# 0xEigenLabs/eigen-zkvm

Hardware: AMD Instinct MI355X
Metric: Goldilocks NTT GElems/s + BN254 G1 MSM Mpts/s; starky prove ms at 2^24 rows (higher is better)
Workload: dtype u64 (Goldilocks, canonical)

## Files before the change

eigen-zkvm_amd/csrc/ntt.hip:

```cpp
#include "zk_internal.h"
#include "ntt_reg.hip.h"
#include <map>
#include <mutex>
#include <type_traits>
#include <vector>

namespace zk {

namespace {

constexpr int NTT_TILE = 4096;
constexpr int TW_LO_BITS = 12;
constexpr int TW_LO = 1 << TW_LO_BITS;

struct PassParams {
    const u64* in;
    u64* out;
    const u64* w256;
    const u64* tw_lo;
    const u64* tw_hi;
    const u64* tw_mid;
    u64 pre_scale;
    u32 dshift;
    const u64* sc_lo;
    const u64* sc_hi;
    u64 sc_step;
    u64 out_scale;
    u64 inner;
    u64 valid_in;
    u64 s_np;
    u32 np;
    u32 log_s;
    u32 has_tw;
};

__device__ __forceinline__ u64 tab2(const u64* __restrict__ lo, const u64* __restrict__ hi, u64 e) {
    return gl::mul_tw_nc(hi[e >> TW_LO_BITS], lo[e & (TW_LO - 1)]);
}

template <int LOGA, int LOGB, bool KMODE, bool INV>
__global__ __launch_bounds__(NTT_TILE / 16) void ntt_pass_kernel(const PassParams P) {
    constexpr int LOGR = LOGA + LOGB, R = 1 << LOGR, RA = 1 << LOGA, RB = 1 << LOGB;
    constexpr int C = NTT_TILE / R;
    constexpr int GA = 16 / RA, GB = 16 / RB;
    constexpr int TG = R / 16;
    constexpr int PAD = KMODE ? 512 / R : 0;
    constexpr int ROW = RB * C + PAD;
    static_assert(LOGR >= 4 && LOGR <= 8 && LOGA <= 4 && LOGB <= 4, "tile shape");
    __shared__ u64 lds[RA * ROW];

    const int t = threadIdx.x;
    const u64 u0 = (u64)blockIdx.x * C;

    {
        const int c = t % C, ta = t / C;
        const u64 u = u0 + c;
        const bool live = u < P.inner;
        u64 x[GA][RA];
        const bool full = u0 + C <= P.inner && (u64)(R - 1) * P.inner + u0 + C <= P.valid_in;
        const u64* __restrict__ base = P.in + (u64)(ta * GA) * P.inner + (live ? u : 0);
        if (full) {
#pragma unroll
            for (int g = 0; g < GA; ++g)
#pragma unroll
                for (int ja = 0; ja < RA; ++ja) x[g][ja] = __builtin_nontemporal_load(&base[(u64)(ja * RB + g) * P.inner]);
        } else {
#pragma unroll
            for (int g = 0; g < GA; ++g)
#pragma unroll
                for (int ja = 0; ja < RA; ++ja) {
                    const u64 off = (u64)(ja * RB + g) * P.inner;
                    const bool ok = live && (u64)(ta * GA) * P.inner + off + u < P.valid_in;
                    const u64 v = __builtin_nontemporal_load(ok ? base + off : P.in);
                    x[g][ja] = ok ? v : 0;
                }
        }
#pragma unroll
        for (int g = 0; g < GA; ++g) ntt_reg<LOGA, INV>(x[g]);
        if (LOGR <= 6 && C >= 64 && LOGB > 0 && P.pre_scale == 1) {
            static_for<0, TG>([&](auto TA) {
                constexpr int ta_c = decltype(TA)::value;
                if (ta == ta_c) {
                    static_for<0, GA>([&](auto GI) {
                        constexpr int g = decltype(GI)::value, jb = ta_c * GA + g;
                        static_for<0, RA>([&](auto KA) {
                            constexpr int ka = decltype(KA)::value;
                            constexpr int e0 = (39 * (64 / (R > 64 ? 64 : R)) * jb * ka) % 192, e = INV ? (192 - e0) % 192 : e0;
                            u64 v = x[g][bitrev_c(ka, LOGA)];
                            if constexpr (e >= 96) v = gl::neg(gl::mul_pow2<e - 96>(v));
                            else v = gl::mul_pow2<e>(v);
                            lds[ka * ROW + jb * C + c] = v;
                        });
                    });
                }
            });
        } else
        {
#pragma unroll
            for (int g = 0; g < GA; ++g) {
                const int jb = ta * GA + g;
#pragma unroll
                for (int ka = 0; ka < RA; ++ka) {
                    u64 v = x[g][bitrev_c(ka, LOGA)];
                    if (LOGB > 0 && ka > 0) v = gl::mul_tw(v, P.w256[(jb * ka) << (8 - LOGR)]);
                    else if (P.pre_scale != 1) v = gl::mul_tw(v, P.pre_scale);
                    lds[ka * ROW + jb * C + c] = v;
                }
            }
        }
    }
    __syncthreads();
    {
        int c, tb;
        if (KMODE) { tb = t % TG; c = t / TG; } else { c = t % C; tb = t / C; }
        const u64 u = u0 + c;
        u64 y[GB][RB];
#pragma unroll
        for (int g = 0; g < GB; ++g) {
            const int ka = tb + g * TG;
#pragma unroll
            for (int jb = 0; jb < RB; ++jb) y[g][jb] = lds[ka * ROW + jb * C + c];
        }
        const u64 uc = u < P.inner ? u : 0;
        u64 p, rem;
        if (P.np == 1) { p = uc >> P.log_s; rem = uc & (((u64)1 << P.log_s) - 1); }
        else if ((P.inner >> 32) == 0) { const u32 p32 = (u32)uc / (u32)P.s_np; p = p32; rem = (u32)uc - p32 * (u32)P.s_np; }
        else
        { p = uc / P.s_np; rem = uc - p * P.s_np; }
        u64 tw[GB][RB];
        if (P.tw_mid) {
            const u32 sh = P.log_s - P.dshift, istep = (((u32)p * RA) << sh) * 8;
#pragma unroll
            for (int g = 0; g < GB; ++g) {
                const u32 ka = tb + g * TG, i0 = (((u32)p * ka) << sh) * 8;
#pragma unroll
                for (int kb = 0; kb < RB; ++kb) tw[g][kb] = *(const u64*)((const char*)P.tw_mid + (u32)(i0 + kb * istep));
            }
        }
#pragma unroll
        for (int g = 0; g < GB; ++g) ntt_reg<LOGB, INV>(y[g]);
        if (u >= P.inner) return;

        auto finish = [&](auto small_c) {
            constexpr bool SMALL = decltype(small_c)::value;
            u64* __restrict__ outp = P.out + p * R * P.s_np + rem;
            const u64 kstride = P.s_np;
            const u32 b0 = ((u32)p * R * (u32)P.s_np + (u32)rem) * 8, bstep = RA * (u32)P.s_np * 8;
            auto put = [&](u32 ka, int kb, u64 v) {
                if constexpr (SMALL) *(u64*)((char*)P.out + (u32)(b0 + ka * (u32)P.s_np * 8 + kb * bstep)) = v;
                else outp[(u64)(RA * kb + ka) * kstride] = v;
            };
            const u64 row_q = !P.sc_lo ? 0 : P.np == 1 ? rem : (P.inner >> 32) == 0 ? (u64)((u32)rem / P.np) : rem / P.np;
            if (P.tw_mid) {
#pragma unroll
                for (int g = 0; g < GB; ++g) {
                    const int ka = tb + g * TG;
#pragma unroll
                    for (int kb = 0; kb < RB; ++kb) {
                        u64 v = y[g][bitrev_c(kb, LOGB)];
                        v = gl::mul_tw(v, tw[g][kb]);
                        put(ka, kb, v);
                    }
                }
                return;
            }
            u64 tw_step = 1;
            if (P.has_tw) tw_step = tab2(P.tw_lo, P.tw_hi, (p * RA) << P.log_s);
#pragma unroll
            for (int g = 0; g < GB; ++g) {
                const int ka = tb + g * TG;
                u64 f = P.out_scale;
                if (P.has_tw) f = tab2(P.tw_lo, P.tw_hi, (p * ka) << P.log_s);
                if (P.sc_lo) f = tab2(P.sc_lo, P.sc_hi, ((u64)ka << P.log_s) + row_q);
                const bool scaled = P.has_tw || P.sc_lo || P.out_scale != 1;
                const u64 fstep = P.sc_lo ? P.sc_step : tw_step;
#pragma unroll
                for (int kb = 0; kb < RB; ++kb) {
                    u64 v = y[g][bitrev_c(kb, LOGB)];
                    if (scaled) {
                        v = gl::mul_tw(v, f);
                        if (kb + 1 < RB) f = gl::mul_tw_nc(f, fstep);
                    }
                    put(ka, kb, v);
                }
            }
        };
        if (((P.inner * R) >> 29) == 0) finish(std::true_type{});
        else finish(std::false_type{});
    }
}

__global__ void ntt_small_kernel(const u64* in, u64* out, u32 np, u32 n_in, u32 n, u64 w, u64 g, u64 cst) {
    const u32 tid = blockIdx.x * blockDim.x + threadIdx.x;
    if (tid >= n * np) return;
    const u32 k = tid / np, c = tid % np;
    const u64 wk = gl::pow(w, k);
    u64 acc = 0, cur = 1;
    for (u32 i = 0; i < n_in; ++i) { acc = gl::add(acc, gl::mul(in[(u64)i * np + c], cur)); cur = gl::mul(cur, wk); }
    out[(u64)k * np + c] = gl::mul(acc, gl::mul(cst, gl::pow(g, k)));
}

struct Tables { DevConst w256, w256s, lo, hi, mid; u32 dshift = 0; };
struct ScaleTables { DevConst lo, hi; };

std::mutex g_mu;
auto& g_tables = *new std::map<std::pair<int, std::pair<u32, int>>, Tables>;
auto& g_scales = *new std::map<std::pair<int, std::pair<u32, u64>>, ScaleTables>;

void two_level(u64 base, u64 cst, u32 nbits, std::vector<u64>& lo, std::vector<u64>& hi) {
    lo.resize(TW_LO);
    u64 c = cst;
    for (int i = 0; i < TW_LO; ++i) { lo[i] = c; c = gl::hmul(c, base); }
    size_t nh = nbits > (u32)TW_LO_BITS ? (size_t)1 << (nbits - TW_LO_BITS) : 1;
    hi.resize(nh);
    u64 step = gl::hpow(base, TW_LO);
    c = 1;
    for (size_t i = 0; i < nh; ++i) { hi[i] = c; c = gl::hmul(c, step); }
}

const Tables& get_tables(u32 nbits, bool inverse) {
    int dev; ZK_HIP(hipGetDevice(&dev));
    std::lock_guard<std::mutex> lk(g_mu);
    auto key = std::make_pair(dev, std::make_pair(nbits, (int)inverse));
    auto it = g_tables.find(key);
    if (it != g_tables.end()) return it->second;
    u64 w = gl::hroot(nbits), w8 = gl::hroot(8);
    if (inverse) { w = gl::hinv(w); w8 = gl::hinv(w8); }
    std::vector<u64> t256(256), lo, hi;
    u64 c = 1;
    for (int i = 0; i < 256; ++i) { t256[i] = c; c = gl::hmul(c, w8); }
    two_level(w, 1, nbits, lo, hi);
    Tables T; T.w256 = DevConst(t256); T.lo = DevConst(lo); T.hi = DevConst(hi);
    if (inverse) {
        const u64 ninv = gl::hinv((1ull << nbits) % GL_P);
        std::vector<u64> t256s(256);
        for (int i = 0; i < 256; ++i) t256s[i] = gl::hmul(t256[i], ninv);
        T.w256s = DevConst(t256s);
    }
    {
        T.dshift = nbits > 16 ? nbits - 16 : 0;
        const size_t nm = (size_t)1 << (nbits - T.dshift);
        std::vector<u64> mid(nm);
        const u64 step = gl::hpow(w, 1ull << T.dshift);
        c = 1;
        for (size_t i = 0; i < nm; ++i) { mid[i] = c; c = gl::hmul(c, step); }
        T.mid = DevConst(mid);
    }
    return g_tables.emplace(key, std::move(T)).first->second;
}

const ScaleTables& get_scale(u32 nbits, u64 g, u64 cst) {
    int dev; ZK_HIP(hipGetDevice(&dev));
    std::lock_guard<std::mutex> lk(g_mu);
    auto key = std::make_pair(dev, std::make_pair(nbits, g));
    auto it = g_scales.find(key);
    if (it != g_scales.end()) return it->second;
    std::vector<u64> lo, hi;
    two_level(g, cst, nbits, lo, hi);
    ScaleTables S; S.lo = DevConst(lo); S.hi = DevConst(hi);
    return g_scales.emplace(key, std::move(S)).first->second;
}

template <int LOGA, int LOGB>
void launch_pass(const PassParams& P, bool kmode, bool inverse, hipStream_t st) {
    constexpr int C = NTT_TILE >> (LOGA + LOGB);
    const u64 blocks = (P.inner + C - 1) / C;
    ZK_REQUIRE(blocks < (1ull << 31), "ntt: grid too large");
    const dim3 g((u32)blocks), b(NTT_TILE / 16);
    const int variant = (kmode ? 2 : 0) | (inverse ? 1 : 0);
#define ZK_PASS(K, I) hipLaunchKernelGGL((ntt_pass_kernel<LOGA, LOGB, K, I>), g, b, 0, st, P)
    switch (variant) {
        case 0: ZK_PASS(false, false); break; case 1: ZK_PASS(false, true); break;
        case 2: ZK_PASS(true, false); break;  default: ZK_PASS(true, true); break;
    }
#undef ZK_PASS
    ZK_HIP(hipGetLastError());
}

void launch_pass_logr(int logr, const PassParams& P, bool kmode, bool inverse, hipStream_t st) {
    switch (logr) {
        case 4: launch_pass<2, 2>(P, kmode, inverse, st); break;
        case 5: launch_pass<3, 2>(P, kmode, inverse, st); break;
        case 6: launch_pass<3, 3>(P, kmode, inverse, st); break;
        case 7: launch_pass<4, 3>(P, kmode, inverse, st); break;
        case 8: launch_pass<4, 4>(P, kmode, inverse, st); break;
        default: throw Error("ntt: unsupported pass radix");
    }
}

std::vector<int> plan(u32 nbits) {
    std::vector<int> r;
    if (nbits < 4) return r;
    int np = (nbits + 7) / 8;
    int base = nbits / np, extra = nbits % np;
    for (int i = 0; i < np; ++i) r.push_back(base + (i < extra ? 1 : 0));
    return r;
}

struct Scale { bool on = false; u64 g = 1, cst = 1; };

void run_transform(const u64* in, u64* a, u64* b,
                   u32 n_pols, u32 nbits, u64 valid_rows, bool inverse, Scale sc, u64 out_scale, hipStream_t st) {
    const u64 n = 1ull << nbits;
    if (nbits < 4) {
        u64 w = gl::hroot(nbits);
        if (inverse) w = gl::hinv(w);
        u64 cst = sc.on ? sc.cst : out_scale;
        u64 g = sc.on ? sc.g : 1;
        u32 total = (u32)(n * n_pols);
        hipLaunchKernelGGL(ntt_small_kernel, dim3((total + 255) / 256), dim3(256), 0, st, in, a, n_pols,
                           (u32)valid_rows, (u32)n, w, g, cst);
        ZK_HIP(hipGetLastError());
        return;
    }
    const std::vector<int> radices = plan(nbits);
    const int np = (int)radices.size();
    const Tables& T = get_tables(nbits, inverse);
    const ScaleTables* S = sc.on ? &get_scale(nbits, sc.g, sc.cst) : nullptr;
    u32 log_s = 0;
    const u64* cur = in;
    for (int i = 0; i < np; ++i) {
        const int logr = radices[i];
        u64* dstbuf = ((np - 1 - i) % 2 == 0) ? a : b;
        const bool last = (i == np - 1);
        PassParams P{};
        P.in = cur; P.out = dstbuf;
        P.w256 = T.w256.u(); P.tw_lo = T.lo.u(); P.tw_hi = T.hi.u();
        P.sc_lo = (last && sc.on) ? S->lo.u() : nullptr;
        P.sc_hi = (last && sc.on) ? S->hi.u() : nullptr;
        const int loga = (logr + 1) / 2;
        P.sc_step = (last && sc.on) ? gl::hpow(sc.g, (1ull << loga) << log_s) : 1;
        P.out_scale = 1; P.pre_scale = 1;
        if (last && !sc.on && out_scale != 1) {
            ZK_REQUIRE(inverse && out_scale == gl::hinv(n % GL_P), "ntt: unsupported constant scaling");
            P.w256 = T.w256s.u(); P.pre_scale = out_scale;
        }
        P.inner = (n >> logr) * n_pols;
        P.valid_in = (i == 0) ? valid_rows * n_pols : n * n_pols;
        P.s_np = ((u64)1 << log_s) * n_pols;
        P.np = n_pols;
        P.log_s = log_s;
        P.has_tw = last ? 0 : 1;
        P.dshift = T.dshift;
        P.tw_mid = (!last && log_s >= T.dshift) ? T.mid.u() : nullptr;
        const bool kmode = P.s_np < 16;
        launch_pass_logr(logr, P, kmode, inverse, st);
        cur = dstbuf;
        log_s += logr;
    }
}

}

int ntt_num_passes(uint32_t nbits) { return nbits < 4 ? 1 : (int)plan(nbits).size(); }

const u64* ntt_w256_table(bool inverse) { return get_tables(8, inverse).w256.u(); }

void ntt_dev(const u64* d_src, u64* d_dst, u64* d_tmp, uint32_t n_pols, uint32_t nbits, bool inverse, hipStream_t st) {
    ZK_REQUIRE(nbits <= 32, "ntt: nbits > 32");
    if (n_pols == 0) return;
    ZK_REQUIRE(d_src != d_dst, "ntt: dst may not alias src");
    u64 out_scale = inverse ? gl::hinv((1ull << nbits) % GL_P) : 1;
    run_transform(d_src, d_dst, d_tmp, n_pols, nbits, 1ull << nbits, inverse, Scale{}, out_scale, st);
}

void lde_dev(const u64* d_src, u64* d_dst, u64* d_tmp, uint32_t n_pols, uint32_t nbits, uint32_t nbits_ext, hipStream_t st) {
    ZK_REQUIRE(nbits_ext <= 32 && nbits <= nbits_ext, "lde: need nbits <= nbits_ext <= 32");
    if (n_pols == 0) return;
    ZK_REQUIRE(d_src != d_dst, "lde: dst may not alias src");
    const u64 n = 1ull << nbits;
    Scale sc; sc.on = true; sc.g = 49; sc.cst = gl::hinv(n % GL_P);
    const int fwd_passes = ntt_num_passes(nbits_ext);
    u64* first_fwd_out = ((fwd_passes - 1) % 2 == 0) ? d_dst : d_tmp;
    u64* coef = (first_fwd_out == d_dst) ? d_tmp : d_dst;
    u64* other = (coef == d_dst) ? d_tmp : d_dst;
    run_transform(d_src, coef, other, n_pols, nbits, n, true, sc, 1, st);
    run_transform(coef, d_dst, d_tmp, n_pols, nbits_ext, n, false, Scale{}, 1, st);
}

}
```

Before: 94.52.

## Share twiddle loads across 16-lane rows via DPP broadcast and prefetch tables early

In the NTT pass kernel, each lane of a 16-lane row now loads one distinct w256 or tw_mid twiddle, and the row gets the value it needs through DPP row broadcasts. This replaces the per-lane redundant table gathers, used when the row shares the same p (s_np a multiple of 16, non-K mode). The twiddle and scale table lookups for the output chain are also issued before the first-stage register NTT and the barrier, so their latency overlaps compute. The cost is extra register pressure from the prefetched values and DPP cross-lane instructions. It also relies on the assumption that all 16 lanes in a row share p.

```diff
diff --git a/eigen-zkvm_amd/csrc/ntt.hip b/eigen-zkvm_amd/csrc/ntt.hip
--- a/eigen-zkvm_amd/csrc/ntt.hip
+++ b/eigen-zkvm_amd/csrc/ntt.hip
@@ -32,10 +32,17 @@
     u32 np;
     u32 log_s;
     u32 has_tw;
+    u32 row_p;
 };
 
-__device__ __forceinline__ u64 tab2(const u64* __restrict__ lo, const u64* __restrict__ hi, u64 e) {
-    return gl::mul_tw_nc(hi[e >> TW_LO_BITS], lo[e & (TW_LO - 1)]);
+__device__ __forceinline__ u32 dpp_opaque(u32 v) { asm volatile("" : "+v"(v)); return v; }
+template <int SRC>
+__device__ __forceinline__ u64 row_bcast(u64 v) {
+    static_assert(SRC >= 0 && SRC < 16, "a lane of the row");
+    const u32 v0 = dpp_opaque((u32)v), v1 = dpp_opaque((u32)(v >> 32));
+    const u32 z0 = dpp_opaque((u32)__builtin_amdgcn_update_dpp(0, (int)v0, 0x150 + SRC, 0xF, 0xF, false));
+    const u32 z1 = dpp_opaque((u32)__builtin_amdgcn_update_dpp(0, (int)v1, 0x150 + SRC, 0xF, 0xF, false));
+    return gl::mk64(z0, z1);
 }
 
 template <int LOGA, int LOGB, bool KMODE, bool INV>
@@ -52,6 +59,49 @@
     const int t = threadIdx.x;
     const u64 u0 = (u64)blockIdx.x * C;
 
+    auto lane_pos = [&](int c, u64& p, u64& rem) {
+        const u64 u = u0 + c, uc = u < P.inner ? u : 0;
+        if (P.np == 1) { p = uc >> P.log_s; rem = uc & (((u64)1 << P.log_s) - 1); }
+        else if ((P.inner >> 32) == 0) { const u32 p32 = (u32)uc / (u32)P.s_np; p = p32; rem = (u32)uc - p32 * (u32)P.s_np; }
+        else
+        { p = uc / P.s_np; rem = uc - p * P.s_np; }
+    };
+    const int cb = KMODE ? t / TG : t % C, tb = KMODE ? t % TG : t / C;
+
+    static_assert(C % 16 == 0 && GA * RA == 16 && GB * RB == 16, "a 16-lane row shares ta and owns 16 table entries");
+    const int r16 = t & 15;
+    const bool shift_a = LOGR <= 6 && C >= 64 && LOGB > 0 && P.pre_scale == 1;
+    u64 wa = 0;
+    u64 wm = 0;
+    const bool row_p = !KMODE && P.row_p;
+    const bool chain_tab = !P.tw_mid && (P.has_tw || P.sc_lo);
+    u64 f0[GB], tw_step = 1, t2h[GB + 1], t2l[GB + 1];
+    auto request_tables = [&]() {
+        if (LOGB > 0 && !shift_a) wa = P.w256[(((t / C) * GA + r16 / RA) * (r16 % RA)) << (8 - LOGR)];
+        if (row_p) {
+            u64 p, rem;
+            lane_pos(cb & ~15, p, rem);
+            const u32 kappa = tb + (r16 / RB) * TG + RA * (r16 % RB);
+            wm = *(const u64*)((const char*)P.tw_mid + (u32)((((u32)p * kappa) << (P.log_s - P.dshift)) * 8));
+        }
+        if (chain_tab) {
+            u64 p, rem;
+            lane_pos(cb, p, rem);
+            const u64 row_q = !P.sc_lo ? 0 : P.np == 1 ? rem : (P.inner >> 32) == 0 ? (u64)((u32)rem / P.np) : rem / P.np;
+            const u64 es = (p * RA) << P.log_s;
+            t2h[GB] = P.has_tw ? P.tw_hi[es >> TW_LO_BITS] : 1; t2l[GB] = P.has_tw ? P.tw_lo[es & (TW_LO - 1)] : 1;
+            const u64* __restrict__ hi = P.sc_lo ? P.sc_hi : P.tw_hi;
+            const u64* __restrict__ lo = P.sc_lo ? P.sc_lo : P.tw_lo;
+#pragma unroll
+            for (int g = 0; g < GB; ++g) {
+                const int ka = tb + g * TG;
+                const u64 e = P.sc_lo ? ((u64)ka << P.log_s) + row_q : (p * ka) << P.log_s;
+                t2h[g] = hi[e >> TW_LO_BITS]; t2l[g] = lo[e & (TW_LO - 1)];
+            }
+        }
+    };
+    u64 tw[GB][RB];
+
     {
         const int c = t % C, ta = t / C;
         const u64 u = u0 + c;
@@ -75,9 +125,10 @@
                     x[g][ja] = ok ? v : 0;
                 }
         }
+        request_tables();
 #pragma unroll
         for (int g = 0; g < GA; ++g) ntt_reg<LOGA, INV>(x[g]);
-        if (LOGR <= 6 && C >= 64 && LOGB > 0 && P.pre_scale == 1) {
+        if (shift_a) {
             static_for<0, TG>([&](auto TA) {
                 constexpr int ta_c = decltype(TA)::value;
                 if (ta == ta_c) {
@@ -96,23 +147,41 @@
             });
         } else
         {
-#pragma unroll
-            for (int g = 0; g < GA; ++g) {
+            static_for<0, GA>([&](auto GI) {
+                constexpr int g = decltype(GI)::value;
                 const int jb = ta * GA + g;
-#pragma unroll
-                for (int ka = 0; ka < RA; ++ka) {
+                static_for<0, RA>([&](auto KA) {
+                    constexpr int ka = decltype(KA)::value;
                     u64 v = x[g][bitrev_c(ka, LOGA)];
-                    if (LOGB > 0 && ka > 0) v = gl::mul_tw(v, P.w256[(jb * ka) << (8 - LOGR)]);
+                    if (LOGB > 0 && ka > 0) v = gl::mul_tw(v, row_bcast<g * RA + ka>(wa));
                     else if (P.pre_scale != 1) v = gl::mul_tw(v, P.pre_scale);
                     lds[ka * ROW + jb * C + c] = v;
-                }
-            }
-        }
+                });
+            });
+        }
+    }
+    auto load_mid = [&]() {
+        u64 p, rem;
+        lane_pos(cb, p, rem);
+        const u32 sh = P.log_s - P.dshift, istep = (((u32)p * RA) << sh) * 8;
+#pragma unroll
+        for (int g = 0; g < GB; ++g) {
+            const u32 ka = tb + g * TG, i0 = (((u32)p * ka) << sh) * 8;
+#pragma unroll
+            for (int kb = 0; kb < RB; ++kb) tw[g][kb] = *(const u64*)((const char*)P.tw_mid + (u32)(i0 + kb * istep));
+        }
+    };
+    if (P.tw_mid && !row_p) load_mid();
+#pragma unroll
+    for (int g = 0; g < GB; ++g) f0[g] = P.out_scale;
+    if (chain_tab) {
+#pragma unroll
+        for (int g = 0; g < GB; ++g) f0[g] = gl::mul_tw_nc(t2h[g], t2l[g]);
+        if (P.has_tw) tw_step = gl::mul_tw_nc(t2h[GB], t2l[GB]);
     }
     __syncthreads();
     {
-        int c, tb;
-        if (KMODE) { tb = t % TG; c = t / TG; } else { c = t % C; tb = t / C; }
+        const int c = cb;
         const u64 u = u0 + c;
         u64 y[GB][RB];
 #pragma unroll
@@ -121,25 +190,21 @@
 #pragma unroll
             for (int jb = 0; jb < RB; ++jb) y[g][jb] = lds[ka * ROW + jb * C + c];
         }
-        const u64 uc = u < P.inner ? u : 0;
+#pragma unroll
+        for (int g = 0; g < GB; ++g) ntt_reg<LOGB, INV>(y[g]);
+        if (row_p) {
+            static_for<0, GB>([&](auto GI) {
+                constexpr int g = decltype(GI)::value;
+                static_for<0, RB>([&](auto KB) {
+                    constexpr int kb = decltype(KB)::value;
+                    u64& v = y[g][bitrev_c(kb, LOGB)];
+                    v = gl::mul_tw(v, row_bcast<g * RB + kb>(wm));
+                });
+            });
+        }
+        if (u >= P.inner) return;
         u64 p, rem;
-        if (P.np == 1) { p = uc >> P.log_s; rem = uc & (((u64)1 << P.log_s) - 1); }
-        else if ((P.inner >> 32) == 0) { const u32 p32 = (u32)uc / (u32)P.s_np; p = p32; rem = (u32)uc - p32 * (u32)P.s_np; }
-        else
-        { p = uc / P.s_np; rem = uc - p * P.s_np; }
-        u64 tw[GB][RB];
-        if (P.tw_mid) {
-            const u32 sh = P.log_s - P.dshift, istep = (((u32)p * RA) << sh) * 8;
-#pragma unroll
-            for (int g = 0; g < GB; ++g) {
-                const u32 ka = tb + g * TG, i0 = (((u32)p * ka) << sh) * 8;
-#pragma unroll
-                for (int kb = 0; kb < RB; ++kb) tw[g][kb] = *(const u64*)((const char*)P.tw_mid + (u32)(i0 + kb * istep));
-            }
-        }
-#pragma unroll
-        for (int g = 0; g < GB; ++g) ntt_reg<LOGB, INV>(y[g]);
-        if (u >= P.inner) return;
+        lane_pos(c, p, rem);
 
         auto finish = [&](auto small_c) {
             constexpr bool SMALL = decltype(small_c)::value;
@@ -150,7 +215,13 @@
                 if constexpr (SMALL) *(u64*)((char*)P.out + (u32)(b0 + ka * (u32)P.s_np * 8 + kb * bstep)) = v;
                 else outp[(u64)(RA * kb + ka) * kstride] = v;
             };
-            const u64 row_q = !P.sc_lo ? 0 : P.np == 1 ? rem : (P.inner >> 32) == 0 ? (u64)((u32)rem / P.np) : rem / P.np;
+            if (row_p) {
+#pragma unroll
+                for (int g = 0; g < GB; ++g)
+#pragma unroll
+                    for (int kb = 0; kb < RB; ++kb) put(tb + g * TG, kb, y[g][bitrev_c(kb, LOGB)]);
+                return;
+            }
             if (P.tw_mid) {
 #pragma unroll
                 for (int g = 0; g < GB; ++g) {
@@ -164,14 +235,10 @@
                 }
                 return;
             }
-            u64 tw_step = 1;
-            if (P.has_tw) tw_step = tab2(P.tw_lo, P.tw_hi, (p * RA) << P.log_s);
 #pragma unroll
             for (int g = 0; g < GB; ++g) {
                 const int ka = tb + g * TG;
-                u64 f = P.out_scale;
-                if (P.has_tw) f = tab2(P.tw_lo, P.tw_hi, (p * ka) << P.log_s);
-                if (P.sc_lo) f = tab2(P.sc_lo, P.sc_hi, ((u64)ka << P.log_s) + row_q);
+                u64 f = f0[g];
                 const bool scaled = P.has_tw || P.sc_lo || P.out_scale != 1;
                 const u64 fstep = P.sc_lo ? P.sc_step : tw_step;
 #pragma unroll
@@ -344,6 +411,7 @@
         P.dshift = T.dshift;
         P.tw_mid = (!last && log_s >= T.dshift) ? T.mid.u() : nullptr;
         const bool kmode = P.s_np < 16;
+        P.row_p = (P.tw_mid && !kmode && P.s_np % 16 == 0) ? 1 : 0;
         launch_pass_logr(logr, P, kmode, inverse, st);
         cur = dstbuf;
         log_s += logr;
```

Result: faster. 97.57, median of 6 (+3.2%).
